# wnma3mz/flearn

Hardware: AMD Instinct MI355X
Metric: device-resident GiB/s, FedAVG N-client weighted tensor reduce; %HBM peak (higher is better)
Workload: dtype fp32; 1 GPU; NS: FedAVG reduce, 100 clients x ResNet-50 state_dict (25,610,152 fp32 / 267 tensors) - the north star's 100 x 25 M headline shape; config=ns, clients=100, params=25610152, layout=resnet50, epilogue=mean, order=reference client order (bit-exact), parallelism=single GPU

## Files before the change

### flearn_amd/csrc/fa_geometry.hpp

```cpp
#pragma once

#include <stdint.h>

#include <initializer_list>

#include "flearn_amd.h"

namespace fa {

enum Family { kFamRows, kFamNarrow, kFamRowmajor, kFamSplitn, kFamBalanced, kFamRowsH16, kFamFoldRows, kFamFoldElem };

struct Plan {
  int family;
  int V, W, D;
  int KG, EPIB;
  bool wide16;
  int64_t grid;
};

constexpr double kRowsBlocksPerCU = 0.75;
constexpr int kPieceChunks = 64;

constexpr int kBalancedV = 4, kBalancedU = 1;

constexpr int kSplitW = 4, kSplitD = 8, kSplitMaxN = 256;

inline int64_t row_chunks(int64_t ncols, int per = 4) { return ((ncols + per - 1) / per + 63) / 64; }

inline int64_t ceil_div(int64_t a, int64_t b) { return (a + b - 1) / b; }

inline int64_t natural_grid(int cus) { return (int64_t)(cus * kRowsBlocksPerCU + 0.5); }

inline int64_t rows_grid_max(int cus) { return (int64_t)cus * 13 / 16; }

inline int64_t one_piece_grid(int64_t chunks, int cus, int forced) {
  int64_t grid = forced > 0 ? forced : natural_grid(cus);
  if (forced <= 0 && chunks > grid * kPieceChunks && chunks <= (int64_t)cus * kPieceChunks)
    grid = ceil_div(chunks, kPieceChunks);
  if (grid < 1) grid = 1;
  if (grid > chunks) grid = chunks;
  return grid;
}

inline bool rowmajor_geometry(int64_t chunks, int cus, int64_t target, int64_t* grid, int* kg) {
  const int64_t lo = 160 < cus ? 160 : cus, hi = cus;
  for (int64_t d = 0; d <= hi - lo; ++d) {
    for (int sgn = 0; sgn < 2; ++sgn) {
      const int64_t g = sgn ? target - d : target + d;
      if (g < lo || g > hi || (d == 0 && sgn)) continue;
      const int64_t k = ceil_div(chunks, g * kPieceChunks);
      if (k < 2) return false;
      for (int c : {4, 3, 2}) {
        if (k % c == 0) {
          *grid = g;
          *kg = c;
          return true;
        }
      }
    }
  }
  return false;
}

inline int kg_for(int64_t k) {
  int best = 4;
  int64_t waste = ceil_div(k, 4) * 4 - k;
  for (int c : {3, 2}) {
    const int64_t wc = ceil_div(k, c) * c - k;
    if (wc < waste) {
      waste = wc;
      best = c;
    }
  }
  return best;
}

inline Plan rowmajor_plan(int mode, int op, int64_t chunks, int64_t grid, int kg) {
  const int64_t k = ceil_div(chunks, grid * kPieceChunks);
  const bool yogi_f64 = op == FA_OP_YOGI && mode != FA_MODE_W32_DIV32;
  const bool wide16 = k >= 6 && (kg <= 3 || (kg == 4 && !yogi_f64));
  const int epib = wide16 && op != FA_OP_MEAN ? 4 : 2;
  return Plan{kFamRowmajor, wide16 ? 16 : 8, wide16 ? 4 : 8, 1, kg, epib, wide16, grid};
}

inline Plan rows_plan(int v, int w, int64_t grid) {
  return Plan{kFamRows, v, w, kPieceChunks / (v * w), 0, 0, false, grid};
}

inline Plan plan_f32_window(int mode, int op, int n, int64_t ncols, int cus, int forced, bool splitn) {
  const int64_t chunks = row_chunks(ncols);
  if (splitn && n >= 2 * kSplitW && n <= kSplitMaxN && chunks < cus)
    return Plan{kFamSplitn, 0, kSplitW, kSplitD, 0, 0, false, chunks};
  if (mode != FA_MODE_W64) {
    if (forced > 0 && chunks > (int64_t)forced * kPieceChunks)
      return rowmajor_plan(mode, op, chunks, forced, kg_for(ceil_div(chunks, (int64_t)forced * kPieceChunks)));
    const bool past = chunks > (int64_t)cus * kPieceChunks;
    int64_t g = 0;
    int kg = 0;
    if (forced <= 0 && chunks > rows_grid_max(cus) * kPieceChunks &&
        rowmajor_geometry(chunks, cus, past ? natural_grid(cus) : rows_grid_max(cus), &g, &kg))
      return rowmajor_plan(mode, op, chunks, g, kg);
  }
  int64_t grid = one_piece_grid(chunks, cus, forced);
  int64_t share = ceil_div(chunks, grid);
  if (share <= 2) {
    return Plan{kFamNarrow, 1, 1, n < 350 ? 16 : n < 700 ? 32 : 40, 0, 0, false, chunks};
  }
  if (op == FA_OP_MEAN) {
    const int W = 4;
    if (forced <= 0) {
      int64_t cap = W;
      while (cap < share) cap *= 2;
      const int64_t g2 = ceil_div(chunks, cap / 2);
      if (cap > W && share * 5 < cap * 3 && g2 <= rows_grid_max(cus)) {
        grid = g2;
        share = ceil_div(chunks, grid);
      }
    }
    int v = 1;
    while (v < 16 && share > v * W) v *= 2;
    return rows_plan(v, W, grid);
  }
  if (share <= 4) return rows_plan(1, 4, grid);
  if (share <= 8) return rows_plan(2, 4, grid);
  if (forced <= 0 && share > 16) {
    const int64_t cap = share <= 32 ? 32 : 64;
    const int64_t g2 = ceil_div(chunks, cap / 2);
    if (share * 5 < cap * 3 && g2 <= rows_grid_max(cus)) return rows_plan(ceil_div(chunks, g2) <= 16 ? 4 : 8, 4, g2);
  }
  return rows_plan(share <= 16 ? 2 : share <= 32 ? 4 : 8, 8, grid);
}

inline int window_count(int op, int64_t ncols) {
  if (op != FA_OP_MEAN) return ncols >= ((int64_t)16 << 20) ? 3 : 1;
  return (ncols >= ((int64_t)8 << 20) && ncols < ((int64_t)16 << 20)) ? 2 : 1;
}

inline int64_t window_width(int64_t ncols, int count) {
  return count <= 1 ? ncols : ceil_div(ncols, count) / 256 * 256 + 256;
}

inline Plan plan_f16_window(int vmax, int64_t ncols, int cus, int forced = 0) {
  const int64_t chunks = row_chunks(ncols, 8);
  const int64_t grid = one_piece_grid(chunks, cus, forced);
  const int64_t share = ceil_div(chunks, grid);
  const int w = share <= 1 ? 1 : 4;
  int v = 1;
  while (v < vmax && share > v * w) v *= 2;
  const int d = v * w >= kPieceChunks ? 1 : (kPieceChunks / (v * w) > 16 ? 16 : kPieceChunks / (v * w));
  return Plan{kFamRowsH16, v, w, d, 0, 0, false, grid};
}

inline int64_t balanced_grid(int64_t chunks, int64_t slots) {
  const int64_t grid = chunks < slots ? chunks : slots;
  return grid > 0 ? grid : 1;
}

constexpr int kFoldW = 4;
inline Plan plan_fold_window(int acc_kind, int64_t ncols, int cus, int forced = 0) {
  if (acc_kind == FA_ACC_F64 || acc_kind == FA_ACC_I64) {
    const int64_t blocks = ceil_div(ncols, 256), cap = forced > 0 ? forced : (int64_t)cus * 4;
    return Plan{kFamFoldElem, 1, 4, 1, 0, 0, false, blocks < 1 ? 1 : (blocks < cap ? blocks : cap)};
  }
  const int64_t chunks = row_chunks(ncols);
  int64_t grid = forced > 0 ? forced : natural_grid(cus);
  if (forced <= 0 && chunks > grid * kPieceChunks && chunks <= rows_grid_max(cus) * kPieceChunks)
    grid = ceil_div(chunks, kPieceChunks);
  if (grid > chunks) grid = chunks;
  if (grid < 1) grid = 1;
  const int64_t share = ceil_div(chunks, grid);
  int v = 1;
  while (v < kPieceChunks / kFoldW && share > v * kFoldW) v *= 2;
  return Plan{kFamFoldRows, v, kFoldW, kPieceChunks / (v * kFoldW), 0, 0, false, grid};
}

constexpr int kTrimW = 4;
constexpr int kTrimMaxClients = FA_TRIM_MAX_CLIENTS;

// ... 136 lines not shown
```

### flearn_amd/csrc/fa_host.hpp

```cpp
#pragma once

#include <hip/hip_runtime.h>

#include <stdint.h>

#include <atomic>
#include <string>
#include <type_traits>

#include "fa_numerics.hpp"
#include "flearn_amd.h"

namespace fa {
namespace host {

inline thread_local std::string g_last_error;

inline int fail(int code, const char* what) {
  g_last_error = what;
  return code;
}

struct LaunchRecord {
  const char* kernel = nullptr;
  int64_t grid = 0;
  int32_t launches = 0;
};
inline thread_local LaunchRecord g_last_launch;

template <class P, typename T, auto... A>
struct Inst {};
template <class HP, auto... A>
struct HInst {};
template <class AT, typename T, auto... X>
struct FInst {};
template <auto... A>
struct TInst {};
template <class T>
struct EInst {};

inline std::string make_kernel_name(const char* family, const std::string& f) {
  std::string out = family;
  const size_t b = f.find("Inst<"), e = f.rfind('>');
  if (b == std::string::npos || e == std::string::npos) return out;
  for (size_t i = b + 4; i <= e; ++i) {
    if (f.compare(i, 4, "fa::") == 0) i += 4;
    if (f[i] != ' ') out += f[i];
  }
  return out;
}

template <class I>
const char* pretty_of() {
  return __PRETTY_FUNCTION__;
}

inline void note_launch(const std::string& kernel, int64_t grid) {
  g_last_launch.kernel = kernel.c_str();
  g_last_launch.grid = grid;
  ++g_last_launch.launches;
}

#define FA_TARGS(...) __VA_ARGS__
#define FA_LAUNCH_AS(Tag, family, targs, grid, block, stream, ...)                                              \
  do {                                                                                                          \
    hipLaunchKernelGGL((family<FA_TARGS targs>), dim3((unsigned)(grid)), dim3(block), 0, stream, __VA_ARGS__);  \
    static const std::string name_ = make_kernel_name(#family, pretty_of<Tag<FA_TARGS targs>>());               \
    note_launch(name_, (int64_t)(grid));                                                                        \
  } while (0)
#define FA_LAUNCH(...) FA_LAUNCH_AS(Inst, __VA_ARGS__)

template <class F>
int with_op(int op, F&& f) {
  switch (op) {
    case FA_OP_MEAN: return f(std::integral_constant<int, FA_OP_MEAN>{});
    case FA_OP_AVGM: return f(std::integral_constant<int, FA_OP_AVGM>{});
    case FA_OP_ADAGRAD: return f(std::integral_constant<int, FA_OP_ADAGRAD>{});
    case FA_OP_YOGI: return f(std::integral_constant<int, FA_OP_YOGI>{});
    case FA_OP_ADAM: return f(std::integral_constant<int, FA_OP_ADAM>{});
    case FA_OP_DYN: return f(std::integral_constant<int, FA_OP_DYN>{});
    default: return fail(FA_ERR_ARG, "unknown epilogue op");
  }
}

constexpr bool kNT = true;

inline int device_cus() {
  static thread_local int dev = -1, cus = 0;
  int d = 0;
  if (hipGetDevice(&d) != hipSuccess) return 256;
  if (d != dev) {
    if (hipDeviceGetAttribute(&cus, hipDeviceAttributeMultiprocessorCount, d) != hipSuccess || cus <= 0)
      cus = 256;
    dev = d;
  }
  return cus;
}

template <typename K>
int resident_blocks_per_cu(K kernel) {
  static int occ = 0;
  if (occ == 0) {
    int o = 0;
    if (hipOccupancyMaxActiveBlocksPerMultiprocessor(&o, kernel, kThreads, 0) != hipSuccess || o <= 0) o = 1;
    occ = o;
  }
  return occ;
}

template <typename X>
bool aligned_window(const X* stack, int64_t stride, int64_t col0) {
  const uintptr_t a = (uintptr_t)(stack + col0);
  return (a % (4 * sizeof(X))) == 0 && ((stride * (int64_t)sizeof(X)) % (4 * sizeof(X))) == 0;
}

inline int launch_check() {
  const hipError_t err = hipGetLastError();
  if (err != hipSuccess) return fail(FA_ERR_LAUNCH, hipGetErrorString(err));
  return FA_OK;
}

inline std::atomic<int> g_reduce_grid{0};

template <class P, typename T>
struct Window {
  const typename P::x_t* stack;
  int64_t stride;
  int n;
  const typename P::w_t* w;
  int64_t col0, ncols;
  Epi<T> e;
};
#define FA_WIN(a) a.stack, a.stride, a.n, a.w, a.col0, a.ncols, a.e

inline int no_kernel(const char* family) {
  return fail(FA_ERR_ARG, (std::string("no shipped ") + family + " instantiation for the plan").c_str());
}

template <typename T>
Epi<T> epi_at(const Epi<T>& e, int64_t c) {
  Epi<T> o = e;
  if (o.prev) o.prev += c;
  if (o.v) o.v += c;
  if (o.v_out) o.v_out += c;
  if (o.h) o.h += c;
  if (o.out32) o.out32 += c;
  if (o.out64) o.out64 += c;
  return o;
}

inline bool aligned_to(const void* p, size_t a) { return ((uintptr_t)p % a) == 0; }

inline bool overlaps(const void* a, const void* b, size_t bytes) {
  const uintptr_t x = (uintptr_t)a, y = (uintptr_t)b;
  return x < y + bytes && y < x + bytes;
}

template <typename T>
int make_epi(const fa_epilogue* in, double denom, int n_reduced, float* out32, double* out64, Epi<T>* e,
             int64_t ncols = 0) {
  e->denom = (T)denom;
  e->prev = nullptr;
  e->v = nullptr;
  e->h = nullptr;
  e->trace = nullptr;
  e->v_out = nullptr;
  e->beta = e->eta = e->tau = e->beta2 = e->c = e->n = T(0);
  e->alpha32 = 0.f;
  e->out32 = out32;
  e->out64 = out64;
  if (!in || in->op == FA_OP_MEAN) return FA_OK;
  if (in->op < FA_OP_AVGM || in->op > FA_OP_DYN) return fail(FA_ERR_ARG, "unknown epilogue op");
  if (!in->v) return fail(FA_ERR_ARG, "epilogue needs v");
  e->v = static_cast<T*>(in->v);
  if (in->v_out) {
    if (!aligned_to(in->v_out, 4 * sizeof(T))) return fail(FA_ERR_ALIGN, "v_out must be 4-element aligned");
    if (in->v_out == in->v || (ncols > 0 && overlaps(in->v_out, in->v, (size_t)ncols * sizeof(T))))
      return fail(FA_ERR_ARG, "v_out must be NULL (in place) or an array not overlapping v");
    e->v_out = static_cast<T*>(in->v_out);
  }
  if (in->op == FA_OP_DYN) {
    if (!in->h) return fail(FA_ERR_ARG, "FedDyn epilogue needs h");
    const double nc = in->n_clients > 0 ? in->n_clients : (double)n_reduced;
    if (!(nc >= 1)) return fail(FA_ERR_ARG, "FedDyn epilogue needs n_clients >= 1");
    e->h = in->h;
    e->n = (T)nc;
    e->c = (T)(in->alpha / nc);
    e->alpha32 = (float)in->alpha;
    return FA_OK;
  }
  if (!in->prev) return fail(FA_ERR_ARG, "epilogue needs prev and v");
  e->prev = in->prev;
  e->beta = (T)in->beta;
  e->eta = (T)in->eta;
  e->tau = (T)in->tau;
  e->beta2 = (T)in->beta2;
  e->c = (T)(1.0 - in->beta2);
  return FA_OK;
}

template <class F>
int with_mode(int mode, const fa_epilogue* epi, double denom, int n_clients, float* out32, double* out64,
              int64_t ncols, F&& f) {
  auto go = [&](auto p, auto t) {
    Epi<decltype(t)> e;
    if (int rc = make_epi(epi, denom, n_clients, out32, out64, &e, ncols)) return rc;
    return f(p, e);
  };
  switch (mode) {
    case FA_MODE_W32_DIV64: return go(AccF32{}, double{});
    case FA_MODE_W32_DIV32: return go(AccF32{}, float{});
    case FA_MODE_W64: return go(AccF32W64{}, double{});
    default: return fail(FA_ERR_ARG, "unknown reduce mode");
  }
}

inline int check_columns(const float* out32, const double* out64, const void* prev, const void* v,
                  size_t v_elem, const float* h = nullptr) {
  if (!aligned_to(out32, 16) || !aligned_to(out64, 32) || !aligned_to(prev, 16) ||
      !aligned_to(v, 4 * v_elem) || !aligned_to(h, 16))
    return fail(FA_ERR_ALIGN, "output / prev / v / h arrays must be 4-element aligned");
  return FA_OK;
}

inline int check_window(const void* stack, int64_t stride, int n, const void* w, int64_t col0, int64_t ncols,
                 bool has_output) {
  if (n <= 0) return fail(FA_ERR_ARG, "n_clients must be >= 1");
  if (ncols < 0 || col0 < 0 || stride < col0 + ncols) return fail(FA_ERR_ARG, "bad column window");
  if (!stack || !w) return fail(FA_ERR_ARG, "null stack or weights");
  if (!has_output) return fail(FA_ERR_ARG, "no output");
  return FA_OK;
}

template <typename X>
int check_common(const X* stack, int64_t stride, int n, const void* w, int64_t col0,
                 int64_t ncols, const void* o1, const void* o2) {
  if (int rc = check_window(stack, stride, n, w, col0, ncols, o1 || o2)) return rc;
  if (!aligned_window(stack, stride, col0)) return fail(FA_ERR_ALIGN, "row window not 16-B aligned");
  return FA_OK;
}

}
}
```

### flearn_amd/csrc/fa_numerics.hpp

```cpp
#pragma once

#include <hip/hip_runtime.h>
#include <stdint.h>

#include "flearn_amd.h"

namespace fa {

constexpr int kThreads = 256;

template <typename T>
struct vec4 {
  typedef T type __attribute__((ext_vector_type(4)));
};

template <typename T, bool NT>
__device__ __forceinline__ typename vec4<T>::type load_quad(const T* p) {
  if constexpr (NT)
    return __builtin_nontemporal_load(reinterpret_cast<const typename vec4<T>::type*>(p));
  else
    return *reinterpret_cast<const typename vec4<T>::type*>(p);
}

template <typename T>
__device__ __forceinline__ typename vec4<T>::type load_quad_guarded(const T* p, int valid) {
  typename vec4<T>::type r = {T(0), T(0), T(0), T(0)};
  if (valid > 0) r[0] = p[0];
  if (valid > 1) r[1] = p[1];
  if (valid > 2) r[2] = p[2];
  if (valid > 3) r[3] = p[3];
  return r;
}

template <typename T>
__device__ __forceinline__ void store_quad(T* p, typename vec4<T>::type v, int valid) {
  if (valid == 4) {
    *reinterpret_cast<typename vec4<T>::type*>(p) = v;
  } else {
    if (valid > 0) p[0] = v[0];
    if (valid > 1) p[1] = v[1];
    if (valid > 2) p[2] = v[2];
  }
}

struct AccF32 {
  typedef float x_t;
  typedef float w_t;
  typedef float acc_t;
  static __device__ __forceinline__ float mul(float w, float x) { return w * x; }
};
struct AccF32W64 {
  typedef float x_t;
  typedef double w_t;
  typedef double acc_t;
  static __device__ __forceinline__ double mul(double w, float x) { return w * (double)x; }
};
struct AccF64 {
  typedef double x_t;
  typedef double w_t;
  typedef double acc_t;
  static __device__ __forceinline__ double mul(double w, double x) { return w * x; }
};
struct AccI64 {
  typedef int64_t x_t;
  typedef int64_t w_t;
  typedef int64_t acc_t;
  static __device__ __forceinline__ int64_t mul(int64_t w, int64_t x) {
    return (int64_t)((uint64_t)w * (uint64_t)x);
  }
};

template <typename A>
__device__ __forceinline__ A add(A a, A b) {
  return a + b;
}
template <>
__device__ __forceinline__ int64_t add<int64_t>(int64_t a, int64_t b) {
  return (int64_t)((uint64_t)a + (uint64_t)b);
}

template <typename T>
struct Epi {
  T denom;
  const float* prev;
  T* v;
  T beta, eta, tau, beta2, c;
  float* h;
  T n;
  float alpha32;
  float* out32;
  double* out64;
  unsigned long long* trace;
  T* v_out;
};

template <typename T>
__device__ __forceinline__ T sign_of(T x) {
  return x > T(0) ? T(1) : (x < T(0) ? T(-1) : (x == T(0) ? T(0) : x));
}

template <typename T, int OP>
__device__ __forceinline__ T update(const Epi<T>& e, T g, T l, T& vv) {
  if constexpr (OP == FA_OP_MEAN) {
    return g;
  } else {
    const T d = g - l;
    if constexpr (OP == FA_OP_AVGM) {
      vv = d + e.beta * vv;
      return l + vv;
    } else {
      const T m = d * d;
      if constexpr (OP == FA_OP_ADAGRAD) {
        vv = vv + m;
      } else if constexpr (OP == FA_OP_YOGI) {
        vv = vv - (e.c * m) * sign_of<T>(vv - m);
      } else {
        vv = e.beta2 * vv + e.c * m;
      }
      return l + (e.eta * d) / (sqrt(vv) + e.tau);
    }
  }
}

template <typename T, int OP, typename A>
__device__ __forceinline__ void epi_compute(const Epi<T>& e, const typename vec4<A>::type a,
                                            typename vec4<float>::type& l, typename vec4<T>::type& vv,
                                            typename vec4<T>::type& w) {
  if constexpr (OP == FA_OP_DYN) {
#pragma unroll
    for (int j = 0; j < 4; ++j) {
      const T g = (T)a[j] / e.denom;
      const T d = g * e.n - vv[j];
      const float hn = (float)((T)l[j] - e.c * d);
      const float ah = e.alpha32 * hn;
      w[j] = g - (T)ah;
      l[j] = hn;
      vv[j] = w[j];
    }
  } else {
#pragma unroll
    for (int j = 0; j < 4; ++j) {
      const T g = (T)a[j] / e.denom;
      T vj = vv[j];
      w[j] = update<T, OP>(e, g, (T)l[j], vj);
      vv[j] = vj;
    }
  }
}

template <typename T, int OP, typename A>
__device__ __forceinline__ void finish_quad(const Epi<T>& e, int64_t c, int valid,
                                            typename vec4<A>::type acc) {
  typename vec4<T>::type w;
  typename vec4<T>::type vv = {T(0), T(0), T(0), T(0)};
  typename vec4<float>::type l = {0.f, 0.f, 0.f, 0.f};
  if constexpr (OP != FA_OP_MEAN) {
    const float* ls = OP == FA_OP_DYN ? e.h : e.prev;
    if (valid == 4) {
      l = *reinterpret_cast<const typename vec4<float>::type*>(ls + c);
      vv = *reinterpret_cast<const typename vec4<T>::type*>(e.v + c);
    } else {
      l = load_quad_guarded(ls + c, valid);
      vv = load_quad_guarded(e.v + c, valid);
    }
  }
  epi_compute<T, OP, A>(e, acc, l, vv, w);
  if constexpr (OP == FA_OP_DYN) store_quad<float>(e.h + c, l, valid);
  if constexpr (OP != FA_OP_MEAN) store_quad<T>((e.v_out ? e.v_out : e.v) + c, vv, valid);
  if (e.out32) {
    typename vec4<float>::type o = {(float)w[0], (float)w[1], (float)w[2], (float)w[3]};
    store_quad<float>(e.out32 + c, o, valid);
  }
  if (e.out64) {
    typename vec4<double>::type o = {(double)w[0], (double)w[1], (double)w[2], (double)w[3]};
    store_quad<double>(e.out64 + c, o, valid);
  }
}

typedef unsigned int u32x4 __attribute__((ext_vector_type(4)));

__device__ __forceinline__ __amdgpu_buffer_rsrc_t row_rsrc(const void* base, uint32_t bytes) {
  return __builtin_amdgcn_make_buffer_rsrc(const_cast<void*>(base), (short)0, (int)bytes, 0x00020000);
}

template <bool NT>
__device__ __forceinline__ vec4<float>::type buf_load_quad(__amdgpu_buffer_rsrc_t r, int voff, int soff) {
  const u32x4 u = __builtin_amdgcn_raw_buffer_load_b128(r, voff, soff, NT ? 2 : 0);
  return __builtin_bit_cast(vec4<float>::type, u);
}

constexpr int kEpiLoadAux = 0;
constexpr int kEpiStoreAux = 2;
constexpr int kEpiStore64Aux = kEpiStoreAux;
template <typename T>
__device__ __forceinline__ typename vec4<T>::type buf_load_tquad(__amdgpu_buffer_rsrc_t r, int q) {
  if constexpr (sizeof(T) == 4) {
    return __builtin_bit_cast(typename vec4<T>::type, __builtin_amdgcn_raw_buffer_load_b128(r, q * 16, 0, kEpiLoadAux));
  } else {
    typedef double d2 __attribute__((ext_vector_type(2)));
    const d2 lo = __builtin_bit_cast(d2, __builtin_amdgcn_raw_buffer_load_b128(r, q * 32, 0, kEpiLoadAux));
    const d2 hi = __builtin_bit_cast(d2, __builtin_amdgcn_raw_buffer_load_b128(r, q * 32 + 16, 0, kEpiLoadAux));
    return typename vec4<T>::type{lo[0], lo[1], hi[0], hi[1]};
  }
}

template <typename T, bool XL = false>
__device__ __forceinline__ void buf_store_tquad(__amdgpu_buffer_rsrc_t r, int q, typename vec4<T>::type v) {
  if constexpr (sizeof(T) == 4) {
    __builtin_amdgcn_raw_buffer_store_b128(__builtin_bit_cast(u32x4, v), r, q * 16, 0, kEpiStoreAux);
  } else if constexpr (XL) {
    typedef double d2 __attribute__((ext_vector_type(2)));
    __shared__ d2 xch[8][128];
    int tid = (int)threadIdx.x;
    asm volatile("" : "+v"(tid));
    const int lane = tid & 63;
    d2* s = xch[tid >> 6];
    s[2 * lane] = d2{v[0], v[1]};
    s[2 * lane + 1] = d2{v[2], v[3]};
    __atomic_signal_fence(__ATOMIC_SEQ_CST);
    __builtin_amdgcn_wave_barrier();
    const d2 a = s[lane], b = s[64 + lane];
    const int base = (q - lane) * 32;
    __builtin_amdgcn_raw_buffer_store_b128(__builtin_bit_cast(u32x4, a), r, base + lane * 16, 0, kEpiStore64Aux);
    __builtin_amdgcn_raw_buffer_store_b128(__builtin_bit_cast(u32x4, b), r, base + 1024 + lane * 16, 0,
                                           kEpiStore64Aux);
    __builtin_amdgcn_wave_barrier();
    __atomic_signal_fence(__ATOMIC_SEQ_CST);
  } else {
    typedef double d2 __attribute__((ext_vector_type(2)));
    const d2 lo = {v[0], v[1]}, hi = {v[2], v[3]};
    __builtin_amdgcn_raw_buffer_store_b128(__builtin_bit_cast(u32x4, lo), r, q * 32, 0, kEpiStore64Aux);
    __builtin_amdgcn_raw_buffer_store_b128(__builtin_bit_cast(u32x4, hi), r, q * 32 + 16, 0, kEpiStore64Aux);
  }
}

template <typename E>
__device__ __forceinline__ __amdgpu_buffer_rsrc_t col_rsrc(E* base, int64_t qbase, int cols) {
  const uint64_t a = (uint64_t)(uintptr_t)base + (uint64_t)(qbase * 4 * (int64_t)sizeof(E));
  const uint32_t lo = (uint32_t)__builtin_amdgcn_readfirstlane((int)(uint32_t)a);
  const uint32_t hi = (uint32_t)__builtin_amdgcn_readfirstlane((int)(uint32_t)(a >> 32));
  const uint32_t n = (uint32_t)__builtin_amdgcn_readfirstlane(base ? cols * (int)sizeof(E) : 0);
  return row_rsrc(reinterpret_cast<const void*>((uintptr_t)(((uint64_t)hi << 32) | lo)), n);
}

template <typename T, int OP>
struct EpiRsrc {
  __amdgpu_buffer_rsrc_t rl, rv, rvo, r32, r64;
  __device__ __forceinline__ EpiRsrc(const Epi<T>& e, int64_t qbase, int cols)
      : rl(col_rsrc<const float>(OP == FA_OP_DYN ? e.h : e.prev, qbase, OP == FA_OP_MEAN ? 0 : cols)),
        rv(col_rsrc<T>(e.v, qbase, OP == FA_OP_MEAN ? 0 : cols)),
        rvo(col_rsrc<T>(e.v_out ? e.v_out : e.v, qbase, OP == FA_OP_MEAN ? 0 : cols)),
        r32(col_rsrc<float>(e.out32, qbase, cols)),
        r64(col_rsrc<double>(e.out64, qbase, cols)) {}
};

template <typename T, int OP>
__device__ __forceinline__ void epi_load(const EpiRsrc<T, OP>& r, int q, typename vec4<float>::type& l,
                                         typename vec4<T>::type& vv) {
  if constexpr (OP != FA_OP_MEAN) {
    l = buf_load_tquad<float>(r.rl, q);
    vv = buf_load_tquad<T>(r.rv, q);
  } else {
    l = typename vec4<float>::type{0.f, 0.f, 0.f, 0.f};
    vv = typename vec4<T>::type{T(0), T(0), T(0), T(0)};
  }
}

template <typename T, int OP, bool GUARD = true, bool XL = false>
__device__ __forceinline__ void epi_store(const Epi<T>& e, const EpiRsrc<T, OP>& r, int q,
                                          const typename vec4<float>::type l, const typename vec4<T>::type vv,
                                          const typename vec4<T>::type w) {
  if constexpr (OP == FA_OP_DYN) buf_store_tquad<float>(r.rl, q, l);
  if constexpr (OP != FA_OP_MEAN) buf_store_tquad<T, XL>(r.rvo, q, vv);
  if (!GUARD || e.out32) buf_store_tquad<float>(r.r32, q, typename vec4<float>::type{(float)w[0], (float)w[1], (float)w[2], (float)w[3]});
  if (!GUARD || e.out64) buf_store_tquad<double, XL>(r.r64, q, typename vec4<double>::type{(double)w[0], (double)w[1], (double)w[2], (double)w[3]});
}

template <typename T, int OP, typename A, bool GUARD = true, bool XL = false>
__device__ __forceinline__ void epi_quad(const Epi<T>& e, const EpiRsrc<T, OP>& r, int q,
                                         const typename vec4<A>::type a, typename vec4<float>::type l,
                                         typename vec4<T>::type vv) {
  typename vec4<T>::type w;
  epi_compute<T, OP, A>(e, a, l, vv, w);
  epi_store<T, OP, GUARD, XL>(e, r, q, l, vv, w);
}

template <typename T, int OP, typename A, int V, int STEP, int B, bool XL = false>
__device__ __forceinline__ void finish_piece(const Epi<T>& e, int64_t qbase, int cols,
                                             const typename vec4<A>::type (&acc)[V]) {
  static_assert(V % B == 0, "batch must divide the slots");
  if (cols <= 0) return;
  const EpiRsrc<T, OP> r(e, qbase, cols);
#pragma unroll
  for (int b0 = 0; b0 < V; b0 += B) {
    typename vec4<float>::type l[B];
    typename vec4<T>::type vv[B];
#pragma unroll
    for (int b = 0; b < B; ++b) epi_load<T, OP>(r, (int)threadIdx.x + (b0 + b) * STEP, l[b], vv[b]);
#pragma unroll
    for (int b = 0; b < B; ++b)
      epi_quad<T, OP, A, true, XL>(e, r, (int)threadIdx.x + (b0 + b) * STEP, acc[b0 + b], l[b], vv[b]);
  }
}

template <class P>
__device__ __forceinline__ typename vec4<typename P::acc_t>::type quad_axpy(
    typename vec4<typename P::acc_t>::type acc, typename P::w_t w, typename vec4<float>::type x) {
  typedef typename vec4<typename P::acc_t>::type AV;
  if constexpr (sizeof(typename P::acc_t) == 4)
    return acc + w * x;
  else
    return acc + (AV)(typename P::acc_t)w * __builtin_convertvector(x, AV);
}
template <class P>
__device__ __forceinline__ typename vec4<typename P::acc_t>::type quad_mul(
    typename P::w_t w, typename vec4<float>::type x) {
  typedef typename vec4<typename P::acc_t>::type AV;
  if constexpr (sizeof(typename P::acc_t) == 4)
    return w * x;
  else
    return (AV)(typename P::acc_t)w * __builtin_convertvector(x, AV);
}

struct StackRows {
  const char* tile0;
  int64_t row_bytes;
  __device__ __forceinline__ const char* operator()(int i) const { return tile0 + (int64_t)i * row_bytes; }
};
struct PtrRows {
  const float* const* __restrict__ ptr;
  int64_t off_bytes;
  __device__ __forceinline__ const char* operator()(int i) const {
    return reinterpret_cast<const char*>(ptr[i]) + off_bytes;
  }
};

template <class P, int V, int D, int W, bool NT, class R>
__device__ __forceinline__ void rows_sweep(const R& row, uint32_t bytes, int n,
                                           const typename P::w_t* __restrict__ w,
                                           typename vec4<typename P::acc_t>::type (&acc)[V],
                                           int voff = (int)threadIdx.x * 16) {
  typedef typename vec4<float>::type XV;
  XV x[D][V];
#pragma unroll
  for (int d = 0; d < D; ++d)
    if (1 + d < n) {
      const __amdgpu_buffer_rsrc_t r = row_rsrc(row(1 + d), bytes);
#pragma unroll
      for (int v = 0; v < V; ++v) x[d][v] = buf_load_quad<NT>(r, voff + v * 64 * W * 16, 0);
    }
  {
    const __amdgpu_buffer_rsrc_t r = row_rsrc(row(0), bytes);
    const typename P::w_t w0 = w[0];
#pragma unroll
    for (int v = 0; v < V; ++v) acc[v] = quad_mul<P>(w0, buf_load_quad<NT>(r, voff + v * 64 * W * 16, 0));
  }
  int i = 1;
  for (; i + 2 * D <= n; i += D) {
#pragma unroll
    for (int d = 0; d < D; ++d) {
      const typename P::w_t wi = w[i + d];
#pragma unroll
      for (int v = 0; v < V; ++v) acc[v] = quad_axpy<P>(acc[v], wi, x[d][v]);
      __builtin_amdgcn_sched_barrier(0);
      const __amdgpu_buffer_rsrc_t r = row_rsrc(row(i + d + D), bytes);
#pragma unroll
      for (int v = 0; v < V; ++v) x[d][v] = buf_load_quad<NT>(r, voff + v * 64 * W * 16, 0);
      __builtin_amdgcn_sched_barrier(0);
    }
  }
#pragma unroll
  for (int d = 0; d < D; ++d) {
    if (i + d < n) {
      const typename P::w_t wi = w[i + d];
#pragma unroll
      for (int v = 0; v < V; ++v) acc[v] = quad_axpy<P>(acc[v], wi, x[d][v]);
      if (i + d + D < n) {
        const __amdgpu_buffer_rsrc_t r = row_rsrc(row(i + d + D), bytes);
#pragma unroll
        for (int v = 0; v < V; ++v) x[d][v] = buf_load_quad<NT>(r, voff + v * 64 * W * 16, 0);
      }
    }
  }
#pragma unroll
  for (int d = 0; d < D; ++d) {
    if (i + D + d < n) {
      const typename P::w_t wi = w[i + D + d];
#pragma unroll
      for (int v = 0; v < V; ++v) acc[v] = quad_axpy<P>(acc[v], wi, x[d][v]);
    }
  }
}

}
```

### flearn_amd/csrc/fa_stack.hpp

```cpp
#pragma once

#include "fa_numerics.hpp"

namespace fa {

enum Part : int {
  kFull = 0,
  kMasked = 1
};

template <class P, typename T, int OP, int V, int U, bool NT, int PART>
__device__ __forceinline__ void reduce_subtile(const typename P::x_t* __restrict__ base,
                                               int64_t stride, int n,
                                               const typename P::w_t* __restrict__ w, int64_t q0,
                                               int nv, const Epi<T>& e) {
  typedef typename P::x_t X;
  typedef typename P::acc_t A;
  typedef typename vec4<X>::type XV;
  typedef typename vec4<A>::type AV;
  const X* lane = base + q0 * 4;
  int off[V];
#pragma unroll
  for (int v = 0; v < V; ++v) off[v] = ((PART == kFull || v < nv) ? v : nv - 1) * kThreads * 4;
  AV acc[V];
// ... 179 lines not shown
        const AV p = quad_mul<P>(ws[i < cnt ? i : 0], x[d]);
        acc = i < cnt ? acc + p : acc;
        aacc = i < cnt ? aacc + absq(p) : aacc;
        __builtin_amdgcn_sched_barrier(0);
        const int r = i + D < cnt ? i + D : cnt - 1;
        x[d] = buf_load_quad<NT>(row_rsrc(tile0 + (int64_t)r * row_bytes, bytes), voff, 0);
        __builtin_amdgcn_sched_barrier(0);
      }
    }
  }
  part[wv][lane] = acc;
  apart[wv][lane] = aacc;
  __syncthreads();
#pragma unroll
  for (int h = 1; h < W; h *= 2) {
    if ((wv % (2 * h)) == 0 && wv + h < W) {
      part[wv][lane] = part[wv][lane] + part[wv + h][lane];
      apart[wv][lane] = apart[wv][lane] + apart[wv + h][lane];
    }
    __syncthreads();
  }
  if (wv == 0) {
    AV r = part[0][lane];
    const AV aa = apart[0][lane];
    bool flag[4], any = false;
#pragma unroll
    for (int k = 0; k < 4; ++k) {
      const A ab = r[k] < A(0) ? -r[k] : r[k];
      flag[k] = !(aa[k] <= A(2) * ab) || !(ab <= A(3.0e38));
      any |= flag[k];
    }
    if (__builtin_amdgcn_ballot_w64(any && lane < nq) != 0) {
      AV seq[1];
      rows_sweep<P, 1, 16, 1, NT>(StackRows{tile00, stride * 4}, bytes, n, w, seq);
#pragma unroll
      for (int k = 0; k < 4; ++k) r[k] = flag[k] ? seq[0][k] : r[k];
    }
    const AV rr[1] = {r};
    finish_piece<T, OP, A, 1, 64, 1>(e, qb, tcols, rr);
  }
}

template <class P, typename T, int OP, int V, int D, int W, bool NT>
__global__ __launch_bounds__(64 * W) void reduce_kernel_rows(const float* __restrict__ stack,
                                                             int64_t stride, int n,
                                                             const typename P::w_t* __restrict__ w,
                                                             int64_t col0, int64_t ncols, Epi<T> e) {
  static_assert(sizeof(typename P::x_t) == 4, "row pipeline is for 4-byte elements");
  const int64_t nquads = (ncols + 3) / 4;
  const int64_t chunks = (nquads + 63) / 64;
  const int64_t g = gridDim.x;
  const int64_t k = (chunks + g * W * V - 1) / (g * W * V);
  const int64_t pc = (chunks + g * k - 1) / (g * k);
  const int64_t pieces = (chunks + pc - 1) / pc;
  for (int64_t p = blockIdx.x; p < pieces; p += g) {
    const int64_t qs = p * pc * 64;
    rows_piece<P, T, OP, V, D, W, NT>(stack, stride, n, w, col0, ncols, e, qs,
                                      qs + pc * 64 < nquads ? qs + pc * 64 : nquads);
  }
}

template <class P, typename T, int OP, int D, int W, bool NT>
__global__ __launch_bounds__(64 * W) void reduce_kernel_narrow(const float* __restrict__ stack, int64_t stride,
                                                               int n, const typename P::w_t* __restrict__ w,
                                                               int64_t col0, int64_t ncols, Epi<T> e) {
  static_assert(sizeof(typename P::x_t) == 4 && D <= 63, "4-byte rows; vmcnt counts 63 loads");
  typedef typename P::acc_t A;
  typedef typename vec4<A>::type AV;
  typedef typename vec4<float>::type XV;
  const int64_t nquads = (ncols + 3) / 4;
  const int64_t qb = (int64_t)blockIdx.x * 64 * W;
  const int64_t qe = qb + 64 * W < nquads ? qb + 64 * W : nquads;
  const int64_t cend = qe * 4 < ncols ? qe * 4 : ncols;
  if (cend <= qb * 4) return;
  const int cols = (int)(cend - qb * 4);
  const uint32_t bytes = (uint32_t)cols * 4u;
  const int voff = (int)threadIdx.x * 16;
  const int64_t rb = stride * 4;
  const char* base = reinterpret_cast<const char*>(stack + col0 + qb * 4);
  const char* lastp = base + (int64_t)(n - 1) * rb;
  const char* p = base + rb;
#define FA_NW_LOAD(dst, CLAMP)                                                         \
  {                                                                                      \
    const char* q_ = p;                                                                  \
    if (CLAMP) q_ = p <= lastp ? p : lastp;                                              \
    dst = buf_load_quad<NT>(row_rsrc(q_, bytes), voff, 0);                               \
    p += rb;                                                                             \
    asm volatile("" : "+s"(p));                                                          \
  }
  typedef typename P::w_t WT;
  const __amdgpu_buffer_rsrc_t wr = row_rsrc(w, (uint32_t)n * (uint32_t)sizeof(WT));
  const int lane = (int)threadIdx.x & 63;
  auto wload = [&](int first) {
    if constexpr (sizeof(WT) == 4)
      return __builtin_bit_cast(WT, __builtin_amdgcn_raw_buffer_load_b32(wr, (lane + first) * 4, 0, 0));
    else
      return __builtin_bit_cast(WT, __builtin_amdgcn_raw_buffer_load_b64(wr, (lane + first) * 8, 0, 0));
  };
  auto wlane = [](WT v, int l) {
    if constexpr (sizeof(WT) == 4) {
      return __builtin_bit_cast(WT, __builtin_amdgcn_readlane(__builtin_bit_cast(int, v), l));
    } else {
      const long long b = __builtin_bit_cast(long long, v);
      const int lo = __builtin_amdgcn_readlane((int)b, l), hi = __builtin_amdgcn_readlane((int)(b >> 32), l);
      return __builtin_bit_cast(WT, (long long)(((unsigned long long)(unsigned)hi << 32) | (unsigned)lo));
    }
  };
  WT wcur = wload(1);
  XV x[D];
#pragma unroll
  for (int d = 0; d < D; ++d) FA_NW_LOAD(x[d], true);
  AV acc = quad_mul<P>(w[0], buf_load_quad<NT>(row_rsrc(base, bytes), voff, 0));
  int i = 1;
  for (; i + 2 * D <= n; i += D) {
    const WT wnext = wload(i + D);
#pragma unroll
    for (int d = 0; d < D; ++d) {
      acc = quad_axpy<P>(acc, wlane(wcur, d), x[d]);
      __builtin_amdgcn_sched_barrier(0);
      FA_NW_LOAD(x[d], false);
      __builtin_amdgcn_sched_barrier(0);
    }
    wcur = wnext;
  }
  for (; i < n; i += D) {
    const WT wnext = wload(i + D);
#pragma unroll
    for (int d = 0; d < D; ++d) {
      const AV t = quad_axpy<P>(acc, wlane(wcur, d), x[d]);
      acc = i + d < n ? t : acc;
      __builtin_amdgcn_sched_barrier(0);
      FA_NW_LOAD(x[d], true);
      __builtin_amdgcn_sched_barrier(0);
    }
    wcur = wnext;
  }
#undef FA_NW_LOAD
  const AV accs[1] = {acc};
  finish_piece<T, OP, A, 1, 64 * W, 1>(e, qb, cols, accs);
}

__device__ __forceinline__ void rowmajor_piece_geom(int64_t g0, int j, int64_t k, int64_t pc, int64_t pieces,
                                                    int64_t nquads, int64_t ncols, int64_t* qb, uint32_t* bytes) {
  const int64_t pj = blockIdx.x + (g0 + j) * (int64_t)gridDim.x;
  int64_t q = pj * pc * 64;
  const int64_t qe = q + pc * 64 < nquads ? q + pc * 64 : nquads;
  const int64_t ce = qe * 4 < ncols ? qe * 4 : ncols;
  const int64_t left = ce - q * 4;
  const uint32_t b = (pj < pieces && g0 + j < k && left > 0) ? (uint32_t)left * 4u : 0u;
  *qb = b ? q : 0;
  *bytes = b;
}

template <class P, typename T, int OP, int V, int D, int W, int KG, bool NT, int EPIB, bool TR, bool XL>
__device__ __forceinline__ void rowmajor_group(const char* __restrict__ base, int64_t row_bytes, int n,
                                               const typename P::w_t* __restrict__ w, int64_t g0, int64_t k,
                                               int64_t pc, int64_t pieces, int64_t nquads, int64_t ncols,
                                               int gi, const Epi<T>& e,
                                               typename vec4<float>::type (&x)[D][V]) {
  static_assert(KG % D == 0, "pipeline depth must divide the group size");
  typedef typename P::acc_t A;
  typedef typename vec4<A>::type AV;
  const int voff = (int)threadIdx.x * 16;
  int64_t qb[KG];
  uint32_t bytes[KG];
#pragma unroll
  for (int j = 0; j < KG; ++j) rowmajor_piece_geom(g0, j, k, pc, pieces, nquads, ncols, &qb[j], &bytes[j]);
  AV acc[KG][V];
#define FA_RM_LOAD(slot, row, j)                                                                      \
  {                                                                                                   \
    const __amdgpu_buffer_rsrc_t r_ = row_rsrc(base + qb[j] * 16 + (int64_t)(row) * row_bytes, bytes[j]); \
    _Pragma("unroll") for (int v = 0; v < V; ++v) x[slot][v] = buf_load_quad<NT>(r_, voff + v * 64 * W * 16, 0); \
  }
#pragma unroll
  for (int d = 0; d < D; ++d) FA_RM_LOAD(d, 0, d);
#pragma unroll
  for (int j = 0; j < KG; ++j) {
    const typename P::w_t w0 = w[0];
#pragma unroll
    for (int v = 0; v < V; ++v) acc[j][v] = quad_mul<P>(w0, x[j % D][v]);
    __builtin_amdgcn_sched_barrier(0);
    if (j + D < KG) {
      FA_RM_LOAD(j % D, 0, j + D);
    } else if (n > 1) {
      FA_RM_LOAD(j % D, 1, j + D - KG);
    }
    __builtin_amdgcn_sched_barrier(0);
  }
  int i = 1;
  for (; i + 1 < n; ++i) {
    const typename P::w_t wi = w[i];
#pragma unroll
    for (int j = 0; j < KG; ++j) {
#pragma unroll
      for (int v = 0; v < V; ++v) acc[j][v] = quad_axpy<P>(acc[j][v], wi, x[j % D][v]);
      __builtin_amdgcn_sched_barrier(0);
      if (j + D < KG) {
        FA_RM_LOAD(j % D, i, j + D);
      } else {
        FA_RM_LOAD(j % D, i + 1, j + D - KG);
      }
      __builtin_amdgcn_sched_barrier(0);
    }
  }
  if (i < n) {
    const typename P::w_t wi = w[i];
#pragma unroll
    for (int j = 0; j < KG; ++j) {
#pragma unroll
      for (int v = 0; v < V; ++v) acc[j][v] = quad_axpy<P>(acc[j][v], wi, x[j % D][v]);
      if (j + D < KG) FA_RM_LOAD(j % D, i, j + D);
    }
  }
#undef FA_RM_LOAD
  if constexpr (TR) {
    if (threadIdx.x == 0 && gi < 7) e.trace[blockIdx.x * 16 + 1 + 2 * gi] = wall_clock64();
  }
#pragma unroll
  for (int j = 0; j < KG; ++j) finish_piece<T, OP, A, V, 64 * W, EPIB, XL>(e, qb[j], (int)(bytes[j] / 4), acc[j]);
  if constexpr (TR) {
    if (threadIdx.x == 0 && gi < 7) e.trace[blockIdx.x * 16 + 2 + 2 * gi] = wall_clock64();
  }
}

template <class P, typename T, int OP, int V, int D, int W, int KG, bool NT, int EPIB = (V >= 2 ? 2 : V),
          bool TR = false, bool XL = (sizeof(T) == 8 && OP != FA_OP_MEAN && KG <= 3)>
__global__ __launch_bounds__(64 * W) void reduce_kernel_rowmajor(const float* __restrict__ stack,
                                                                 int64_t stride, int n,
                                                                 const typename P::w_t* __restrict__ w,
                                                                 int64_t col0, int64_t ncols, Epi<T> e) {
  static_assert(sizeof(typename P::x_t) == 4, "row pipeline is for 4-byte elements");
  const int64_t nquads = (ncols + 3) / 4;
  const int64_t chunks = (nquads + 63) / 64;
  const int64_t g = gridDim.x;
  const int64_t k = (chunks + g * W * V - 1) / (g * W * V);
  const int64_t pc = (chunks + g * k - 1) / (g * k);
  const int64_t pieces = (chunks + pc - 1) / pc;
  const int64_t row_bytes = stride * 4;
  const char* base = reinterpret_cast<const char*>(stack + col0);
  if constexpr (TR) {
    if (threadIdx.x == 0) e.trace[blockIdx.x * 16] = wall_clock64();
  }
  static_assert(EPIB >= 1, "the piece epilogue batches at least one slot");
  typename vec4<float>::type x[D][V];
  int gi = 0;
  for (int64_t g0 = 0; g0 < k; g0 += KG)
    rowmajor_group<P, T, OP, V, D, W, KG, NT, EPIB, TR, XL>(base, row_bytes, n, w, g0, k, pc, pieces, nquads, ncols,
                                                            gi++, e, x);
}

}
```

Baseline: 6740 GiB/s.

## Replace fp64 mean division with exact reciprocal multiply and overlap quotients with tail loads

Result: faster. 6834 GiB/s, median of 6 (+1.4%).

```diff
diff --git a/flearn_amd/csrc/fa_geometry.hpp b/flearn_amd/csrc/fa_geometry.hpp
--- a/flearn_amd/csrc/fa_geometry.hpp
+++ b/flearn_amd/csrc/fa_geometry.hpp
@@ -1,6 +1,7 @@
 #pragma once
 
 #include <stdint.h>
+#include <string.h>
 
 #include <initializer_list>
 
@@ -24,6 +25,15 @@
 constexpr int kBalancedV = 4, kBalancedU = 1;
 
 constexpr int kSplitW = 4, kSplitD = 8, kSplitMaxN = 256;
+
+inline bool recip_quot_exact(double d) {
+  uint64_t u;
+  memcpy(&u, &d, sizeof u);
+  const int exp = (int)((u >> 52) & 0x7ff) - 1023;
+  if (exp < -100 || exp > 100) return false;
+  if (exp == 100 && (u & 0xfffffffffffffull) != 0) return false;
+  return (u & ((1ull << 26) - 1)) == 0;
+}
 
 inline int64_t row_chunks(int64_t ncols, int per = 4) { return ((ncols + per - 1) / per + 63) / 64; }
 
diff --git a/flearn_amd/csrc/fa_host.hpp b/flearn_amd/csrc/fa_host.hpp
--- a/flearn_amd/csrc/fa_host.hpp
+++ b/flearn_amd/csrc/fa_host.hpp
@@ -8,6 +8,7 @@
 #include <string>
 #include <type_traits>
 
+#include "fa_geometry.hpp"
 #include "fa_numerics.hpp"
 #include "flearn_amd.h"
 
@@ -160,6 +161,8 @@
 int make_epi(const fa_epilogue* in, double denom, int n_reduced, float* out32, double* out64, Epi<T>* e,
              int64_t ncols = 0) {
   e->denom = (T)denom;
+  e->rq = sizeof(T) == 8 && recip_quot_exact(denom) ? 1 : 0;
+  e->rdenom = e->rq ? 1.0 / denom : 0.0;
   e->prev = nullptr;
   e->v = nullptr;
   e->h = nullptr;
diff --git a/flearn_amd/csrc/fa_numerics.hpp b/flearn_amd/csrc/fa_numerics.hpp
--- a/flearn_amd/csrc/fa_numerics.hpp
+++ b/flearn_amd/csrc/fa_numerics.hpp
@@ -92,7 +92,27 @@
   double* out64;
   unsigned long long* trace;
   T* v_out;
-};
+  double rdenom;
+  int rq;
+};
+
+template <typename T, typename A>
+constexpr bool kHasRecipQuot = sizeof(T) == 8 && sizeof(A) == 4;
+
+template <typename T, typename A, int RQ>
+__device__ __forceinline__ T quot(const Epi<T>& e, A a) {
+  if constexpr (RQ != 0 && kHasRecipQuot<T, A>) {
+    const double x = (double)a, d = (double)e.denom;
+    const double q0 = x * e.rdenom;
+#ifdef FA_TUNE_QUOT_MUL
+    if constexpr (RQ == 2) return q0;
+#endif
+    const double q = __builtin_fma(__builtin_fma(-q0, d, x), e.rdenom, q0);
+    return (q0 == 0.0 || !__builtin_isfinite(q0)) ? q0 : q;
+  } else {
+    return (T)a / e.denom;
+  }
+}
 
 template <typename T>
 __device__ __forceinline__ T sign_of(T x) {
@@ -122,14 +142,14 @@
   }
 }
 
-template <typename T, int OP, typename A>
+template <typename T, int OP, typename A, int RQ = 0>
 __device__ __forceinline__ void epi_compute(const Epi<T>& e, const typename vec4<A>::type a,
                                             typename vec4<float>::type& l, typename vec4<T>::type& vv,
                                             typename vec4<T>::type& w) {
   if constexpr (OP == FA_OP_DYN) {
 #pragma unroll
     for (int j = 0; j < 4; ++j) {
-      const T g = (T)a[j] / e.denom;
+      const T g = quot<T, A, RQ>(e, a[j]);
       const T d = g * e.n - vv[j];
       const float hn = (float)((T)l[j] - e.c * d);
       const float ah = e.alpha32 * hn;
@@ -140,7 +160,7 @@
   } else {
 #pragma unroll
     for (int j = 0; j < 4; ++j) {
-      const T g = (T)a[j] / e.denom;
+      const T g = quot<T, A, RQ>(e, a[j]);
       T vj = vv[j];
       w[j] = update<T, OP>(e, g, (T)l[j], vj);
       vv[j] = vj;
@@ -276,13 +296,28 @@
   if (!GUARD || e.out64) buf_store_tquad<double, XL>(r.r64, q, typename vec4<double>::type{(double)w[0], (double)w[1], (double)w[2], (double)w[3]});
 }
 
-template <typename T, int OP, typename A, bool GUARD = true, bool XL = false>
+template <typename T, int OP, typename A, bool GUARD = true, bool XL = false, int RQ = 0>
 __device__ __forceinline__ void epi_quad(const Epi<T>& e, const EpiRsrc<T, OP>& r, int q,
                                          const typename vec4<A>::type a, typename vec4<float>::type l,
                                          typename vec4<T>::type vv) {
   typename vec4<T>::type w;
-  epi_compute<T, OP, A>(e, a, l, vv, w);
+  epi_compute<T, OP, A, RQ>(e, a, l, vv, w);
   epi_store<T, OP, GUARD, XL>(e, r, q, l, vv, w);
+}
+
+template <typename T, int OP, typename A, int V, int STEP, int B, bool XL, int RQ>
+__device__ __forceinline__ void finish_piece_rq(const Epi<T>& e, const EpiRsrc<T, OP>& r,
+                                                const typename vec4<A>::type (&acc)[V]) {
+#pragma unroll
+  for (int b0 = 0; b0 < V; b0 += B) {
+    typename vec4<float>::type l[B];
+    typename vec4<T>::type vv[B];
+#pragma unroll
+    for (int b = 0; b < B; ++b) epi_load<T, OP>(r, (int)threadIdx.x + (b0 + b) * STEP, l[b], vv[b]);
+#pragma unroll
+    for (int b = 0; b < B; ++b)
+      epi_quad<T, OP, A, true, XL, RQ>(e, r, (int)threadIdx.x + (b0 + b) * STEP, acc[b0 + b], l[b], vv[b]);
+  }
 }
 
 template <typename T, int OP, typename A, int V, int STEP, int B, bool XL = false>
@@ -291,16 +326,13 @@
   static_assert(V % B == 0, "batch must divide the slots");
   if (cols <= 0) return;
   const EpiRsrc<T, OP> r(e, qbase, cols);
-#pragma unroll
-  for (int b0 = 0; b0 < V; b0 += B) {
-    typename vec4<float>::type l[B];
-    typename vec4<T>::type vv[B];
-#pragma unroll
-    for (int b = 0; b < B; ++b) epi_load<T, OP>(r, (int)threadIdx.x + (b0 + b) * STEP, l[b], vv[b]);
-#pragma unroll
-    for (int b = 0; b < B; ++b)
-      epi_quad<T, OP, A, true, XL>(e, r, (int)threadIdx.x + (b0 + b) * STEP, acc[b0 + b], l[b], vv[b]);
-  }
+  if constexpr (OP == FA_OP_MEAN && kHasRecipQuot<T, A>) {
+    if (e.rq == 1) return finish_piece_rq<T, OP, A, V, STEP, B, XL, 1>(e, r, acc);
+#ifdef FA_TUNE_QUOT_MUL
+    if (e.rq == 2) return finish_piece_rq<T, OP, A, V, STEP, B, XL, 2>(e, r, acc);
+#endif
+  }
+  finish_piece_rq<T, OP, A, V, STEP, B, XL, 0>(e, r, acc);
 }
 
 template <class P>
diff --git a/flearn_amd/csrc/fa_stack.hpp b/flearn_amd/csrc/fa_stack.hpp
--- a/flearn_amd/csrc/fa_stack.hpp
+++ b/flearn_amd/csrc/fa_stack.hpp
@@ -355,7 +355,8 @@
   *bytes = b;
 }
 
-template <class P, typename T, int OP, int V, int D, int W, int KG, bool NT, int EPIB, bool TR, bool XL>
+template <class P, typename T, int OP, int V, int D, int W, int KG, bool NT, int EPIB, bool TR, bool XL,
+          bool EARLY = false, int RQ = 0>
 __device__ __forceinline__ void rowmajor_group(const char* __restrict__ base, int64_t row_bytes, int n,
                                                const typename P::w_t* __restrict__ w, int64_t g0, int64_t k,
                                                int64_t pc, int64_t pieces, int64_t nquads, int64_t ncols,
@@ -364,7 +365,8 @@
   static_assert(KG % D == 0, "pipeline depth must divide the group size");
   typedef typename P::acc_t A;
   typedef typename vec4<A>::type AV;
-  const int voff = (int)threadIdx.x * 16;
+  int voff = (int)threadIdx.x * 16;
+  if constexpr (EARLY) asm volatile("" : "+v"(voff));
   int64_t qb[KG];
   uint32_t bytes[KG];
 #pragma unroll
@@ -406,6 +408,8 @@
       __builtin_amdgcn_sched_barrier(0);
     }
   }
+  static_assert(!EARLY || (OP == FA_OP_MEAN && sizeof(A) == 4), "early quotients: the plain fp32 mean");
+  constexpr int kQB = V >= 2 ? 2 : 1;
   if (i < n) {
     const typename P::w_t wi = w[i];
 #pragma unroll
@@ -413,17 +417,70 @@
 #pragma unroll
       for (int v = 0; v < V; ++v) acc[j][v] = quad_axpy<P>(acc[j][v], wi, x[j % D][v]);
       if (j + D < KG) FA_RM_LOAD(j % D, i, j + D);
+      if constexpr (EARLY) {
+        if (j + 1 < KG) {
+#pragma unroll
+          for (int v0 = 0; v0 < V; v0 += kQB) {
+            __builtin_amdgcn_sched_barrier(0);
+#pragma unroll
+            for (int v = v0; v < v0 + kQB; ++v)
+#pragma unroll
+              for (int c = 0; c < 4; ++c) acc[j][v][c] = (A)quot<T, A, RQ>(e, acc[j][v][c]);
+          }
+          __builtin_amdgcn_sched_barrier(0);
+        }
+      }
     }
   }
 #undef FA_RM_LOAD
   if constexpr (TR) {
     if (threadIdx.x == 0 && gi < 7) e.trace[blockIdx.x * 16 + 1 + 2 * gi] = wall_clock64();
   }
-#pragma unroll
-  for (int j = 0; j < KG; ++j) finish_piece<T, OP, A, V, 64 * W, EPIB, XL>(e, qb[j], (int)(bytes[j] / 4), acc[j]);
+  if constexpr (EARLY) {
+#pragma unroll
+    for (int j = 0; j + 1 < KG; ++j) {
+      const __amdgpu_buffer_rsrc_t r32 = col_rsrc<float>(e.out32, qb[j], (int)(bytes[j] / 4));
+#pragma unroll
+      for (int v = 0; v < V; ++v) buf_store_tquad<float>(r32, (int)threadIdx.x + v * 64 * W, acc[j][v]);
+    }
+    if (bytes[KG - 1] > 0) {
+      const EpiRsrc<T, OP> r(e, qb[KG - 1], (int)(bytes[KG - 1] / 4));
+      finish_piece_rq<T, OP, A, V, 64 * W, EPIB, XL, RQ>(e, r, acc[KG - 1]);
+    }
+  } else {
+#pragma unroll
+    for (int j = 0; j < KG; ++j) finish_piece<T, OP, A, V, 64 * W, EPIB, XL>(e, qb[j], (int)(bytes[j] / 4), acc[j]);
+  }
   if constexpr (TR) {
     if (threadIdx.x == 0 && gi < 7) e.trace[blockIdx.x * 16 + 2 + 2 * gi] = wall_clock64();
   }
+}
+
+template <class P, typename T, int OP, int V, int D, int W, int KG, bool NT, int EPIB, bool TR, bool XL, bool ED>
+__device__ __forceinline__ void rowmajor_groups(const char* __restrict__ base, int64_t row_bytes, int n,
+                                                const typename P::w_t* __restrict__ w, int64_t k, int64_t pc,
+                                                int64_t pieces, int64_t nquads, int64_t ncols, const Epi<T>& e,
+                                                typename vec4<float>::type (&x)[D][V]) {
+  typedef typename P::acc_t A;
+  int gi = 0;
+#define FA_RM_GROUPS(EARLY, RQ)                                                                               \
+  for (int64_t g0 = 0; g0 < k; g0 += KG)                                                                      \
+    rowmajor_group<P, T, OP, V, D, W, KG, NT, EPIB, TR, XL, EARLY, RQ>(base, row_bytes, n, w, g0, k, pc, pieces, \
+                                                                       nquads, ncols, gi++, e, x);
+  if constexpr (ED && OP == FA_OP_MEAN && kHasRecipQuot<T, A> && KG <= 3) {
+    if (n >= 2 && e.out64 == nullptr && e.rq == 1) {
+      FA_RM_GROUPS(true, 1)
+      return;
+    }
+#ifdef FA_TUNE_QUOT_MUL
+    if (n >= 2 && e.out64 == nullptr && e.rq == 2) {
+      FA_RM_GROUPS(true, 2)
+      return;
+    }
+#endif
+  }
+  FA_RM_GROUPS(false, 0)
+#undef FA_RM_GROUPS
 }
 
 template <class P, typename T, int OP, int V, int D, int W, int KG, bool NT, int EPIB = (V >= 2 ? 2 : V),
@@ -446,10 +503,7 @@
   }
   static_assert(EPIB >= 1, "the piece epilogue batches at least one slot");
   typename vec4<float>::type x[D][V];
-  int gi = 0;
-  for (int64_t g0 = 0; g0 < k; g0 += KG)
-    rowmajor_group<P, T, OP, V, D, W, KG, NT, EPIB, TR, XL>(base, row_bytes, n, w, g0, k, pc, pieces, nquads, ncols,
-                                                            gi++, e, x);
-}
-
-}
+  rowmajor_groups<P, T, OP, V, D, W, KG, NT, EPIB, TR, XL, true>(base, row_bytes, n, w, k, pc, pieces, nquads, ncols, e, x);
+}
+
+}
```
